# meilisearch/arroy

Measured on AMD Instinct MI355X. Metric: distances/sec, Q=1 batched 768-dim cosine scan (GB/s vs HBM roofline in `roofline`); tree-build seconds at 10M vectors in `build_10m`, higher is better.
Workload: dtype f32; 1 GPU; 1M x 768 cosine Q=1 scan (configs[1])

## Files before the change

### arroy_amd/csrc/dense_device.h

```cpp
#pragma once

namespace ah {

typedef _Float16 f16x8_t __attribute__((ext_vector_type(8)));
typedef float f32x16_t __attribute__((ext_vector_type(16)));
typedef float f32x4_t __attribute__((ext_vector_type(4)));

constexpr uint32_t kDM = 256;
template <int WN>
struct DenseShape {
    static constexpr uint32_t kBN = 64u * WN;
    static constexpr uint32_t kThreads = 128u * WN;
    static constexpr uint32_t kWaves = 2u * WN;
    static constexpr uint32_t kStage = (kDM + kBN) * 128u;
    static constexpr uint32_t kPiecesA = 32u / kWaves, kPiecesB = (kBN / 8u) / kWaves;
};
constexpr uint32_t kDenseHalf = 128;
constexpr uint32_t kDensePitch = kDM + 4;
constexpr uint32_t kDenseLds = kDenseHalf * kDensePitch * 4;
constexpr uint32_t kDenseGroup = 8;
static_assert(2 * DenseShape<4>::kStage <= kDenseLds && 2 * DenseShape<2>::kStage <= kDenseLds, "stage buffers fit");

constexpr uint32_t kSideUndecided = 2u;
constexpr uint32_t kSideVerify = 4u;

struct DenseArgs {
    const uint16_t *rows;
    const float4 *stats;
    const float *headers;
    uint64_t n;
    uint32_t hpitch;
    const uint8_t *shadow;
    uint64_t hstride;
    uint32_t n_cols;
    const FNode *nodes;
    const uint32_t *node_of;
    uint8_t *side_bytes;
    float gamma_s, gamma_r;
    uint32_t n_row_tiles, n_col_tiles, group, verify;
};

template <int WN>
__device__ __forceinline__ void dense_stage(const uint8_t *const (&a_src)[DenseShape<WN>::kPiecesA],
                                            const uint8_t *const (&b_src)[DenseShape<WN>::kPiecesB], uint32_t kb, uint8_t *stage,
                                            uint32_t wave) {
    typedef DenseShape<WN> SH;
    const uint64_t koff = (uint64_t)kb * 128u;
#pragma unroll
    for (uint32_t i = 0; i < SH::kPiecesA; i++)
        __builtin_amdgcn_global_load_lds((const __attribute__((address_space(1))) void *)(a_src[i] + koff),
                                         (__attribute__((address_space(3))) void *)(stage + (i * SH::kWaves + wave) * 1024u), 16, 0,
                                         0);
#pragma unroll
    for (uint32_t i = 0; i < SH::kPiecesB; i++)
        __builtin_amdgcn_global_load_lds(
            (const __attribute__((address_space(1))) void *)(b_src[i] + koff),
            (__attribute__((address_space(3))) void *)(stage + kDM * 128u + (i * SH::kWaves + wave) * 1024u), 16, 0, 0);
}

__device__ __forceinline__ bool dense_block_map(uint32_t b, uint32_t group, uint32_t n_col_tiles, uint32_t n_row_tiles,
                                                uint32_t &rt, uint32_t &ct) {
    const uint32_t xcd = b & 7u, slot = b >> 3;
    const uint32_t per_group = group * n_col_tiles;
    const uint32_t grp = slot / per_group, within = slot % per_group;
    ct = within / group;
    rt = (grp * group + within % group) * 8u + xcd;
    return rt < n_row_tiles;
}
__global__ void k_dense_coverage(uint32_t group, uint32_t n_col_tiles, uint32_t n_row_tiles, uint32_t *__restrict__ counts) {
    uint32_t rt, ct;
    if (!dense_block_map(blockIdx.x, group, n_col_tiles, n_row_tiles, rt, ct)) return;
    if (threadIdx.x == 0) atomicAdd(&counts[(uint64_t)rt * n_col_tiles + ct], 1u);
}

template <int METRIC, int WN>
__global__ __launch_bounds__(DenseShape<WN>::kThreads, 1) void k_forest_dense_screen(DenseArgs a, const AbortFlags abort_flag) {
    typedef DenseShape<WN> SH;
    extern __shared__ uint4 s_dense4[];
    uint8_t *smem = reinterpret_cast<uint8_t *>(s_dense4);
    if (abort_requested(abort_flag)) return;
    uint32_t rt, ct;
    if (!dense_block_map(blockIdx.x, a.group, a.n_col_tiles, a.n_row_tiles, rt, ct)) return;
    const uint64_t row0 = (uint64_t)rt * kDM;
    const uint32_t c0 = ct * SH::kBN;
    const uint32_t wave = threadIdx.x >> 6, lane = threadIdx.x & 63u;

    const uint8_t *a_src[SH::kPiecesA], *b_src[SH::kPiecesB];
    {
        const uint32_t sl = lane & 7u;
#pragma unroll
        for (uint32_t i = 0; i < SH::kPiecesA; i++) {
            const uint32_t R = (i * SH::kWaves + wave) * 8u + (lane >> 3);
            const uint64_t r = min(row0 + R, a.n - 1);
            a_src[i] = reinterpret_cast<const uint8_t *>(a.rows) + r * ((uint64_t)a.hpitch * 2u) + ((sl ^ ((R >> 1) & 7u)) << 4);
        }
#pragma unroll
        for (uint32_t i = 0; i < SH::kPiecesB; i++) {
            const uint32_t R = (i * SH::kWaves + wave) * 8u + (lane >> 3);
            const uint32_t c = min(c0 + R, a.n_cols - 1);
            b_src[i] = a.shadow + (uint64_t)c * a.hstride + ((sl ^ ((R >> 1) & 7u)) << 4);
        }
    }
    const uint32_t wm = wave / WN, wn = wave % WN;
    const uint32_t m = lane & 31u, g = lane >> 5, swz = (m >> 1) & 7u;
    f32x16_t acc[4][2];
#pragma unroll
    for (int im = 0; im < 4; im++)
#pragma unroll
        for (int jn = 0; jn < 2; jn++)
#pragma unroll
            for (int e = 0; e < 16; e++) acc[im][jn][e] = 0.0f;

    const uint32_t nk = a.hpitch >> 6;
    dense_stage<WN>(a_src, b_src, 0, smem, wave);
    for (uint32_t kb = 0; kb < nk; kb++) {
        asm volatile("s_waitcnt vmcnt(0)" ::: "memory");
        __syncthreads();
        if (kb + 1 < nk) dense_stage<WN>(a_src, b_src, kb + 1, smem + ((kb + 1) & 1u) * SH::kStage, wave);
        const uint8_t *st = smem + (kb & 1u) * SH::kStage;
        const uint8_t *sa = st + (wm * 128u + m) * 128u;
        const uint8_t *sb = st + (kDM + wn * 64u + m) * 128u;
#pragma unroll
        for (uint32_t q = 0; q < 4; q++) {
            const uint32_t off = ((2u * q + g) ^ swz) << 4;
            f16x8_t af[4], bf[2];
#pragma unroll
            for (int im = 0; im < 4; im++) af[im] = *reinterpret_cast<const f16x8_t *>(sa + im * 32 * 128 + off);
#pragma unroll
            for (int jn = 0; jn < 2; jn++) bf[jn] = *reinterpret_cast<const f16x8_t *>(sb + jn * 32 * 128 + off);
#pragma unroll
            for (int im = 0; im < 4; im++)
#pragma unroll
                for (int jn = 0; jn < 2; jn++)
                    acc[im][jn] = __builtin_amdgcn_mfma_f32_32x32x16_f16(af[im], bf[jn], acc[im][jn], 0, 0, 0);
        }
    }
    float *S = reinterpret_cast<float *>(smem);
    const uint32_t r_in = threadIdx.x & (kDM - 1u), part = threadIdx.x / kDM;
    constexpr uint32_t kParts = SH::kThreads / kDM;
    const uint64_t row = row0 + r_in;
    const bool live = row < a.n;
    float4 rs = make_float4(0.f, 0.f, 0.f, 0.f);
    float row_extra = 0.0f;
    if (live) {
        rs = a.stats[row];
        if (METRIC == AH_DOT_PRODUCT) row_extra = a.headers[2 * row];
    }
#pragma unroll 1
    for (uint32_t h = 0; h < SH::kBN / kDenseHalf; h++) {
        const uint32_t c_lo = c0 + h * kDenseHalf;
        if (c_lo >= a.n_cols) break;
        __syncthreads();
        if ((wn >> 1) == h) {
#pragma unroll
            for (int im = 0; im < 4; im++)
#pragma unroll
                for (int jn = 0; jn < 2; jn++) {
                    const uint32_t col = (wn & 1u) * 64u + (uint32_t)jn * 32u + m;
#pragma unroll
                    for (int qq = 0; qq < 4; qq++) {
                        const uint32_t rr = wm * 128u + (uint32_t)im * 32u + 8u * (uint32_t)qq + 4u * g;
                        *reinterpret_cast<float4 *>(S + col * kDensePitch + rr) = make_float4(
                            acc[im][jn][4 * qq], acc[im][jn][4 * qq + 1], acc[im][jn][4 * qq + 2], acc[im][jn][4 * qq + 3]);
                    }
                }
        }
        __syncthreads();
        const uint32_t c_hi = min(c_lo + kDenseHalf, a.n_cols) - 1u;
        const uint32_t t_lo = a.nodes[c_lo].tree, t_hi = a.nodes[c_hi].tree;
        for (uint32_t t = t_lo + 8u * part; t <= t_hi; t += 8u * kParts) {
            uint32_t nd[8];
#pragma unroll
            for (uint32_t u = 0; u < 8; u++)
                nd[u] = (live && t + u <= t_hi) ? a.node_of[(uint64_t)(t + u) * a.n + row] : 0xFFFFFFFFu;
#pragma unroll
            for (uint32_t u = 0; u < 8; u++) {
                const uint32_t c = nd[u] - c_lo;
                if (nd[u] != 0xFFFFFFFFu && c < kDenseHalf) {
                    const float s = S[c * kDensePitch + r_in];
                    const NormalStats ns =
                        *reinterpret_cast<const NormalStats *>(a.shadow + (uint64_t)nd[u] * a.hstride + (uint64_t)a.hpitch * 2u);
                    uint32_t side;
                    const bool decided = screen_decides<METRIC>(s, rs, ns, row_extra, a.gamma_s, a.gamma_r, side);
                    a.side_bytes[(uint64_t)(t + u) * a.n + row] =
                        (uint8_t)(decided ? (a.verify ? (kSideVerify | side) : side) : kSideUndecided);
                }
            }
        }
    }
}

#ifndef AH_NARROW_SETS
#define AH_NARROW_SETS 3u
#endif
#ifndef AH_NARROW_PRELOAD
#define AH_NARROW_PRELOAD 1
#endif
constexpr uint32_t kNarrowWaves = 5;
constexpr uint32_t kNarrowRows = 32u * kNarrowWaves;
constexpr uint32_t kNarrowThreads = 64u * (kNarrowWaves + 1u);
template <int NT>
struct NarrowShape {
    static constexpr uint32_t kCT = 32u * NT;
    static constexpr uint32_t kStage = kCT * 128u;
    static constexpr uint32_t kStages = 3;
    static constexpr uint32_t kPieces = kCT / 8u;
    static constexpr uint32_t kEpiWave = 32u * 36u * 4u;
    static constexpr uint32_t kRing = kStages * kStage > kNarrowWaves * kEpiWave ? kStages * kStage : kNarrowWaves * kEpiWave;
    static constexpr uint32_t kLds = kRing + kCT * 16u;
};

template <int METRIC, int NT, bool STREAM>
__global__ __launch_bounds__(kNarrowThreads, 2) void k_forest_dense_narrow(DenseArgs a, const AbortFlags abort_flag) {
    typedef NarrowShape<NT> SH;
    extern __shared__ uint4 s_dense4[];
    uint8_t *smem = reinterpret_cast<uint8_t *>(s_dense4);
    if (abort_requested(abort_flag)) return;
    uint32_t rt, ct;
    if (!dense_block_map(blockIdx.x, a.group, a.n_col_tiles, a.n_row_tiles, rt, ct)) return;
    const uint32_t wave = threadIdx.x >> 6, lane = threadIdx.x & 63u;
    const uint32_t c0 = ct * SH::kCT;
    const uint32_t nk = a.hpitch >> 6;
    if (wave == kNarrowWaves) {
        const uint8_t *b_src[SH::kPieces];
#pragma unroll
        for (uint32_t p = 0; p < SH::kPieces; p++) {
            const uint32_t R = p * 8u + (lane >> 3);
            const uint32_t c = min(c0 + R, a.n_cols - 1);
            b_src[p] = a.shadow + (uint64_t)c * a.hstride + (((lane & 7u) ^ ((R >> 1) & 7u)) << 4);
        }
        {
            NormalStats *nst_all = reinterpret_cast<NormalStats *>(smem + SH::kRing);
#pragma unroll
            for (uint32_t h = 0; h < SH::kCT / 64u; h++)
                nst_all[64u * h + lane] = *reinterpret_cast<const NormalStats *>(
                    a.shadow + (uint64_t)min(c0 + 64u * h + lane, a.n_cols - 1) * a.hstride + (uint64_t)a.hpitch * 2u);
        }
#define AH_NARROW_DMA(KB, SET)                                                                                            \
    _Pragma("unroll") for (uint32_t p_ = 0; p_ < SH::kPieces; p_++) __builtin_amdgcn_global_load_lds(                     \
        (const __attribute__((address_space(1))) void *)(b_src[p_] + (uint64_t)(KB) * 128u),                              \
        (__attribute__((address_space(3))) void *)(smem + (SET) * SH::kStage + p_ * 1024u), 16, 0, 0)
        AH_NARROW_DMA(0, 0);
        if (nk > 1) AH_NARROW_DMA(1, 1);
        for (uint32_t kb = 0; kb < nk; kb++) {
            if (kb + 1 < nk) asm volatile("s_waitcnt vmcnt(%0)" ::"n"(SH::kPieces) : "memory");
            else asm volatile("s_waitcnt vmcnt(0)" ::: "memory");
            __builtin_amdgcn_s_barrier();
            asm volatile("" ::: "memory");
            if (kb + 2 < nk) {
                const uint32_t set = (kb + 2) % 3u;
                AH_NARROW_DMA(kb + 2, set);
            }
        }
#undef AH_NARROW_DMA
        __builtin_amdgcn_s_barrier();
        return;
    }
    const uint32_t m = lane & 15u, kg = lane >> 4;
    const uint64_t row_base = (uint64_t)rt * kNarrowRows + wave * 32u;
    const uint4 *a_src[2];
#pragma unroll
    for (uint32_t i = 0; i < 2; i++)
        a_src[i] = reinterpret_cast<const uint4 *>(reinterpret_cast<const uint8_t *>(a.rows) +
                                                  min(row_base + 16u * i + m, a.n - 1) * ((uint64_t)a.hpitch * 2u) + 16u * kg);
    f32x4_t acc[2][2 * NT];
#pragma unroll
    for (int i = 0; i < 2; i++)
#pragma unroll
        for (int j = 0; j < 2 * NT; j++) acc[i][j] = f32x4_t{0.0f, 0.0f, 0.0f, 0.0f};
    const uint32_t er = lane & 31u, eh = lane >> 5;
    const uint64_t row = row_base + er;
    const bool live = row < a.n;
    float4 rs = make_float4(0.f, 0.f, 0.f, 0.f);
    float row_extra = 0.0f;
    const uint32_t T0 = a.nodes[c0].tree, T1 = a.nodes[min(c0 + SH::kCT, a.n_cols) - 1u].tree;
    uint32_t nd0[8];
#define AH_NARROW_LOAD_ND0()                                                                                              \
    _Pragma("unroll") for (uint32_t u = 0; u < 8; u++) {                                                                  \
        const uint32_t t = T0 + eh + 2u * u;                                                                              \
        const uint32_t v = a.node_of[(uint64_t)min(t, T1) * a.n + min(row, a.n - 1)];                                     \
        nd0[u] = (live && t <= T1) ? v : 0xFFFFFFFFu;        \
    }
    {
        const uint64_t r = min(row, a.n - 1);
        rs = a.stats[r];
        if (METRIC == AH_DOT_PRODUCT) row_extra = a.headers[2 * r];
    }
#if AH_NARROW_PRELOAD
    AH_NARROW_LOAD_ND0()
#endif
    constexpr uint32_t kSets = NT == 2 ? AH_NARROW_SETS : 3u, kAhead = kSets - 1u;
    uint4 ar[kSets][4];
#define AH_NARROW_ISSUE(KB, SET)                                                                                          \
    _Pragma("unroll") for (int i_ = 0; i_ < 4; i_++) ar[SET][i_] =                                                        \
        STREAM ? ld_stream_u4(a_src[i_ >> 1] + (uint64_t)(KB) * 8u + 4u * (i_ & 1))                                       \
               : a_src[i_ >> 1][(uint64_t)(KB) * 8u + 4u * (i_ & 1)]
#define AH_NARROW_STEP(SET, STEADY)                                                                                       \
    if (STEADY || kb + (SET) < nk) {                                                                                      \
        asm volatile("s_waitcnt lgkmcnt(0)" ::: "memory");              \
        __builtin_amdgcn_s_barrier();                                                                                     \
        asm volatile("" ::: "memory");                                                                                    \
        if (STEADY || kb + (SET) + kAhead < nk) AH_NARROW_ISSUE(kb + (SET) + kAhead, ((SET) + kAhead) % kSets);           \
        __builtin_amdgcn_sched_barrier(0);        \
        const uint8_t *sb_ = smem + ((kb + (SET)) % SH::kStages) * SH::kStage + m * 128u;                                 \
        _Pragma("unroll") for (uint32_t s_ = 0; s_ < 2; s_++) {                                                           \
            const f16x8_t a0_ = __builtin_bit_cast(f16x8_t, ar[SET][s_]);                                                 \
            const f16x8_t a1_ = __builtin_bit_cast(f16x8_t, ar[SET][2 + s_]);                                             \
            _Pragma("unroll") for (int j_ = 0; j_ < 2 * NT; j_++) {                                                       \
                                                  \
                const f16x8_t b_ = *reinterpret_cast<const f16x8_t *>(sb_ + j_ * 2048 + (((4u * s_ + kg) ^ ((m >> 1) & 7u)) << 4)); \
                acc[0][j_] = __builtin_amdgcn_mfma_f32_16x16x32_f16(a0_, b_, acc[0][j_], 0, 0, 0);                        \
                acc[1][j_] = __builtin_amdgcn_mfma_f32_16x16x32_f16(a1_, b_, acc[1][j_], 0, 0, 0);                        \
            }                                                                                                             \
        }                                                                                                                 \
    }
#pragma unroll
    for (uint32_t p = 0; p < kAhead; p++) AH_NARROW_ISSUE(min(p, nk - 1u), p);
    uint32_t kb = 0;
    for (; kb + 2u * kSets - 1u <= nk; kb += kSets) {
        AH_NARROW_STEP(0, true)
        AH_NARROW_STEP(1, true)
        AH_NARROW_STEP(2, true)
        if (kSets == 4) AH_NARROW_STEP(kSets - 1, true)
    }
    for (; kb < nk; kb += kSets) {
        AH_NARROW_STEP(0, false)
        AH_NARROW_STEP(1, false)
        AH_NARROW_STEP(2, false)
        if (kSets == 4) AH_NARROW_STEP(kSets - 1, false)
    }
#undef AH_NARROW_STEP
#undef AH_NARROW_ISSUE
    asm volatile("s_waitcnt lgkmcnt(0)" ::: "memory");
    __builtin_amdgcn_s_barrier();
    asm volatile("" ::: "memory");
#if !AH_NARROW_PRELOAD
    AH_NARROW_LOAD_ND0()
#endif
#undef AH_NARROW_LOAD_ND0
    float *S = reinterpret_cast<float *>(smem + wave * SH::kEpiWave);
    const NormalStats *nst_all = reinterpret_cast<const NormalStats *>(smem + SH::kRing);
// ... 156 lines not shown
```

### arroy_amd/csrc/forest.hip

```cpp
#include <algorithm>
#include <atomic>
#include <chrono>
#include <condition_variable>
#include <deque>
#include <array>
#include <thread>
#include <type_traits>
#include <unordered_map>
#include <cstdlib>
#include <immintrin.h>
#include <sys/mman.h>
#include <sys/syscall.h>
#include <unistd.h>
#include <new>

#include "common.h"
#include "split_device.h"
#include "screen_device.h"
#include "level_plan.h"
#include "encode.h"
#include "node_codec.h"

namespace ah {

// ... 2187 lines not shown
            }
            cv.notify_all();
        }
        if (ev[0]) (void)hipEventDestroy(ev[0]);
        if (ev[1]) (void)hipEventDestroy(ev[1]);
        if (cs) (void)hipStreamDestroy(cs);
    }
    void push(void *dst, const void *src, size_t bytes) {
        if (!bytes) return;
        if (inline_mode) {
            const hipError_t e = hipMemcpy(dst, src, bytes, hipMemcpyDeviceToHost);
            if (e != hipSuccess && err == hipSuccess) err = e;
            return;
        }
        {
            std::lock_guard<std::mutex> lk(mu);
            q.push_back(Job{dst, src, bytes, nullptr});
            pending++;
        }
        cv.notify_all();
    }
    void push_stream(StreamJob *job, const void *src) {
        if (job->nodes.empty()) {
            delete job;
            return;
        }
        if (inline_mode) {
            hipStream_t cs = nullptr;
            hipEvent_t ev[2] = {nullptr, nullptr};
            hipError_t e = create_copy_stream(&cs);
            if (e == hipSuccess) e = hipEventCreateWithFlags(&ev[0], hipEventDisableTiming);
            if (e == hipSuccess) e = hipEventCreateWithFlags(&ev[1], hipEventDisableTiming);
            if (e == hipSuccess) e = deliver(*job, reinterpret_cast<const uint8_t *>(src), cs, ev);
            if (e != hipSuccess && err == hipSuccess) err = e;
            if (ev[0]) (void)hipEventDestroy(ev[0]);
            if (ev[1]) (void)hipEventDestroy(ev[1]);
            if (cs) (void)hipStreamDestroy(cs);
            delete job;
            return;
        }
        {
            std::lock_guard<std::mutex> lk(mu);
            q.push_back(Job{nullptr, src, 1, job});
            pending++;
        }
        cv.notify_all();
    }
    hipError_t drain() {
        std::unique_lock<std::mutex> lk(mu);
        cv.wait(lk, [this] { return pending == 0; });
        return err;
    }
    ~Readback() {
        if (!started) return;
        {
            std::lock_guard<std::mutex> lk(mu);
            stop = true;
        }
        cv.notify_all();
        th.join();
    }
};

namespace {
struct LevelBufs {
    DataView dv;
    ScreenView sv;
    int metric, device;
    hipStream_t s;
    uint64_t N;
    uint32_t n_trees, n_nodes, n_tiles;
    FNode *nodes;
    FTile *tiles;
    uint32_t *perm;
    uint8_t *normals;
    uint64_t nstride, hdr_off;
    uint8_t *shadow;
    uint64_t hstride;
    uint8_t *shadow8;
    uint64_t stride8;
    uint64_t *masks;
    uint32_t *tile_left, *node_of;
    uint8_t *side_bytes;
    uint32_t *side_bits;
    ScreenCounters *counters;
    AbortFlags abort_all, abort_gated;
    uint32_t verify;
};

template <class F>
int with_metric(int metric, F &&f) {
    return with_metric_of<AH_EUCLIDEAN, AH_MANHATTAN, AH_COSINE, AH_DOT_PRODUCT>(metric, f);
}

int launch_create_split(const LevelBufs &b, int metric, unsigned grid, size_t cs_shared) {
    return with_metric(metric, [&](auto m) -> int {
        constexpr int M = decltype(m)::value;
        AH_TRY(lds_opt_in(reinterpret_cast<const void *>(k_forest_create_split<M>), b.device, cs_shared));
        hipLaunchKernelGGL(k_forest_create_split<M>, dim3(grid), dim3(64), cs_shared, b.s, b.dv, b.nodes, b.n_nodes, b.perm, b.N,
                           b.normals, b.nstride, b.hdr_off, b.abort_gated.gate);
        return AH_OK;
    });
}

template <int M, int TC, bool LDS>
int launch_screen_rows_inst(const LevelBufs &b, const RowsLaunch &l, const RowsSchedule &sch, unsigned grid, size_t sh, size_t lds_grant) {
    const unsigned threads = LDS ? (TC >= 16 ? 512u : 1024u) : (unsigned)kBlock;
    if (LDS) AH_TRY(lds_opt_in(reinterpret_cast<const void *>(k_forest_screen_rows<M, TC, LDS>), b.device, lds_grant));
    hipLaunchKernelGGL((k_forest_screen_rows<M, TC, LDS>), dim3(grid), dim3(threads), LDS ? sh : 0, b.s, b.dv, b.sv, b.node_of,
                       l.t0, l.np, b.normals, b.nstride, b.hdr_off, b.shadow, b.hstride, b.side_bytes, sch, b.abort_all,
                       b.counters, b.verify);
    return AH_OK;
}
int launch_screen_rows(const LevelBufs &b, const RowsLaunch &l, bool lds, const RowsSchedule &sch, unsigned grid, size_t sh,
                       size_t lds_grant) {
    return with_metric(b.metric, [&](auto m) -> int {
        constexpr int M = decltype(m)::value;
        if (lds) return l.tcv >= 16 ? launch_screen_rows_inst<M, 16, true>(b, l, sch, grid, sh, lds_grant)
                                    : launch_screen_rows_inst<M, 8, true>(b, l, sch, grid, sh, lds_grant);
        switch (l.tcv) {
        case 16: return launch_screen_rows_inst<M, 16, false>(b, l, sch, grid, sh, lds_grant);
        case 8: return launch_screen_rows_inst<M, 8, false>(b, l, sch, grid, sh, lds_grant);
        case 4: return launch_screen_rows_inst<M, 4, false>(b, l, sch, grid, sh, lds_grant);
        default: return launch_screen_rows_inst<M, 2, false>(b, l, sch, grid, sh, lds_grant);
        }
    });
}
}

namespace {
struct DensePlan {
    uint32_t n_row_tiles, n_col_tiles, group;
    bool wide;
    int narrow;
    bool stream;
    uint32_t tile_rows, tile_cols, threads, lds;
    uint64_t grid;
};
DensePlan dense_plan(uint64_t N, uint32_t n_cols) {
    DensePlan p{};
    const long long narrow_max = tun(TUN_DENSE_NARROW_MAX_COLS), narrow_force = tun(TUN_DENSE_NARROW);
    p.narrow = narrow_force == 0 || (long long)n_cols > narrow_max ? 0 : (n_cols <= 64 ? 2 : 4);
    if (p.narrow) {
        p.tile_rows = kNarrowRows;
        p.tile_cols = 32u * (uint32_t)p.narrow;
        p.threads = kNarrowThreads;
        p.lds = p.narrow == 2 ? NarrowShape<2>::kLds : NarrowShape<4>::kLds;
        p.wide = false;
    } else {
        p.wide = n_cols > 128;
        p.tile_rows = kDM;
        p.tile_cols = p.wide ? 256u : 128u;
        p.threads = p.wide ? DenseShape<4>::kThreads : DenseShape<2>::kThreads;
        p.lds = kDenseLds;
    }
    p.n_row_tiles = (uint32_t)((N + p.tile_rows - 1) / p.tile_rows);
    p.n_col_tiles = (n_cols + p.tile_cols - 1) / p.tile_cols;
    p.group = p.n_col_tiles > 1 ? (p.narrow ? 12u : kDenseGroup) : 1u;
    const long long st = tun(TUN_DENSE_NARROW_STREAM);
    p.stream = p.narrow && (st < 0 ? p.n_col_tiles == 1 : st != 0);
    const uint64_t r8 = (p.n_row_tiles + 7) / 8;
    p.grid = 8 * ((r8 + p.group - 1) / p.group) * p.group * p.n_col_tiles;
    return p;
}
unsigned exact_pairs_grid(uint64_t N, uint32_t n_trees) {
    return (unsigned)std::min<uint64_t>((((N + 1023) / 1024 + 7) / 8) * 8 * ((n_trees + 3) / 4), 1u << 16);
}
}

namespace {
struct RowsPlan {
    RowsSchedule sch{};
    unsigned threads = kBlock;
    bool xcd = false, nt = false;
    std::vector<std::pair<uint32_t, unsigned>> launches;
};
int plan_rows_launches(uint64_t N, uint32_t hpitch, uint32_t tcv, uint32_t groups, bool lds, uint64_t group_normal_bytes,
                       RowsPlan *plan) {
    const uint32_t env_rpb = (uint32_t)std::max<long long>(0, tun(TUN_ROWS_PER_BLOCK)) / 32u * 32u;
    const uint32_t rpb = lds ? 1024u : env_rpb ? env_rpb : 32u;
    const uint64_t hrow = (uint64_t)hpitch * 2;
    const uint64_t want_rows = tun(TUN_ROWS_CHUNK_ROWS) > 0 ? (uint64_t)tun(TUN_ROWS_CHUNK_ROWS)
                                                             : ((uint64_t)std::max<long long>(1, tun(TUN_ROWS_CHUNK_MB)) << 20) / hrow;
    uint32_t chunk_rows = (uint32_t)std::max<uint64_t>(rpb, want_rows / rpb * rpb);
    if (chunk_rows > N) chunk_rows = (uint32_t)((N + rpb - 1) / rpb * rpb);
    const uint32_t n_chunks = (uint32_t)((N + chunk_rows - 1) / chunk_rows);
    RowsSchedule &sch = plan->sch;
    sch.n_groups = groups;
    sch.tiles = chunk_rows / rpb;
    sch.chunk_rows = chunk_rows;
    sch.rows_per_block = rpb;
    plan->xcd = !lds && tun(TUN_ROWS_XCD) != 0 && tcv <= 4 && groups >= (uint32_t)std::max<long long>(1, tun(TUN_ROWS_XCD_MIN_GROUPS));
    sch.xcd_slots = plan->xcd ? (groups + 7) / 8 : 0u;
    const uint64_t per_chunk = plan->xcd ? 8ull * sch.xcd_slots * sch.tiles : (uint64_t)groups * sch.tiles;
    const long long nt_force = tun(TUN_ROWS_NT);
    plan->nt = plan->xcd && (nt_force >= 0 ? nt_force != 0 : group_normal_bytes > (uint64_t)std::max<long long>(0, tun(TUN_ROWS_NT_BYTES)));
    if (plan->nt) sch.xcd_slots |= 0x80000000u;
    plan->threads = lds ? (tcv >= 16 ? 512u : 1024u) : (unsigned)kBlock;
    const uint64_t max_items = (uint64_t)std::min<long long>(0xFFFFFFFFll, std::max<long long>(1, tun(TUN_LAUNCH_MAX_ITEMS)));
    AH_REQUIRE(per_chunk * plan->threads <= max_items, AH_ERR_INVALID_ARGUMENT, "forest build: too many trees for one row-major launch");
    const uint32_t chunks_per_launch = (uint32_t)std::min<uint64_t>(n_chunks, (max_items / plan->threads) / per_chunk);
    plan->launches.clear();
    for (uint32_t c0 = 0; c0 < n_chunks; c0 += chunks_per_launch)
        plan->launches.emplace_back(c0, (unsigned)((uint64_t)std::min<uint32_t>(chunks_per_launch, n_chunks - c0) * per_chunk));
    return AH_OK;
}
}

namespace {
template <int M, int WN>
int launch_dense_wide(const LevelBufs &b, const DensePlan &dp, const DenseArgs &da) {
    AH_TRY(lds_opt_in(reinterpret_cast<const void *>(k_forest_dense_screen<M, WN>), b.device, kDenseLds));
    hipLaunchKernelGGL((k_forest_dense_screen<M, WN>), dim3((unsigned)dp.grid), dim3(DenseShape<WN>::kThreads), kDenseLds, b.s, da,
                       b.abort_all);
    return AH_OK;
}
template <int M, int NT>
int launch_dense_narrow(const LevelBufs &b, const DensePlan &dp, const DenseArgs &da) {
    if (dp.stream)
        hipLaunchKernelGGL((k_forest_dense_narrow<M, NT, true>), dim3((unsigned)dp.grid), dim3(kNarrowThreads), NarrowShape<NT>::kLds,
                           b.s, da, b.abort_all);
    else
        hipLaunchKernelGGL((k_forest_dense_narrow<M, NT, false>), dim3((unsigned)dp.grid), dim3(kNarrowThreads), NarrowShape<NT>::kLds,
                           b.s, da, b.abort_all);
    return AH_OK;
}
int launch_dense(const LevelBufs &b, const DensePlan &dp, bool exact_wide, ah_build_stats &st) {
    DenseArgs da{};
    da.rows = b.sv.rows;
    da.stats = b.sv.stats;
    da.headers = b.dv.headers;
    da.n = b.N;
    da.hpitch = b.sv.hpitch;
    da.shadow = b.shadow;
    da.hstride = b.hstride;
    da.n_cols = b.n_nodes;
    da.nodes = b.nodes;
    da.node_of = b.node_of;
    da.side_bytes = b.side_bytes;
    da.gamma_s = (float)(2.0 * ((double)b.sv.hpitch + (double)b.sv.hpitch / 16 + 16.0) * 1.1920929e-7);
    da.gamma_r = b.sv.gamma_r;
    da.n_row_tiles = dp.n_row_tiles;
    da.n_col_tiles = dp.n_col_tiles;
    da.group = dp.group;
    da.verify = b.verify;
    AH_REQUIRE(dp.grid < 0x7FFFFFFFull, AH_ERR_INVALID_ARGUMENT, "forest build: too many tiles for one launch");
    const unsigned egrid = exact_pairs_grid(b.N, b.n_trees);
    AH_TRY(with_metric(b.metric, [&](auto m) -> int {
        constexpr int M = decltype(m)::value;
        if (dp.narrow == 2) AH_TRY((launch_dense_narrow<M, 2>(b, dp, da)));
        else if (dp.narrow == 4) AH_TRY((launch_dense_narrow<M, 4>(b, dp, da)));
        else if (dp.wide) AH_TRY((launch_dense_wide<M, 4>(b, dp, da)));
        else AH_TRY((launch_dense_wide<M, 2>(b, dp, da)));
        if (exact_wide)
            hipLaunchKernelGGL((k_forest_exact_pairs<M, true>), dim3(egrid), dim3(256), 0, b.s, b.dv, b.node_of, b.side_bytes,
                               b.n_trees, b.normals, b.nstride, b.hdr_off, b.counters, b.abort_all);
        else
            hipLaunchKernelGGL((k_forest_exact_pairs<M>), dim3(egrid), dim3(256), 0, b.s, b.dv, b.node_of, b.side_bytes, b.n_trees,
                               b.normals, b.nstride, b.hdr_off, b.counters, b.abort_all);
        return AH_OK;
    }));
    st.dense_launches++;
    st.dense_columns += b.n_nodes;
    return AH_OK;
}

int launch_rows_screened(const LevelBufs &b, const LevelPlan &plan, uint64_t nodes_per_tree, uint64_t rec_bytes,
                         const uint32_t *d_tree_first, size_t lds_grant, ah_build_stats &st) {
    const bool lds = plan.lds_tc != 0;
    const size_t lds_sh = (size_t)plan.lds_worst * rec_bytes;
    for (const RowsLaunch &l : plan.launches) {
        RowsPlan rp;
        AH_TRY(plan_rows_launches(b.N, b.sv.hpitch, l.tcv, l.groups, lds, (uint64_t)l.tcv * nodes_per_tree * rec_bytes, &rp));
        rp.sch.tree_first = d_tree_first;
        for (const auto &c : rp.launches) {
            rp.sch.chunk0 = c.first;
            AH_TRY(launch_screen_rows(b, l, lds, rp.sch, c.second, lds_sh, lds_grant));
        }
        st.margin_mode_launches[lds ? (l.tcv >= 16 ? MM_LDS16 : MM_LDS8) : mm_rows(l.tcv)]++;
        st.rows_xcd_launches += rp.xcd ? rp.launches.size() : 0;
        st.rows_nt_launches += rp.nt ? rp.launches.size() : 0;
        st.rows_split_launches += rp.launches.size() - 1;
    }
    return AH_OK;
}

template <int M, int TC>
int launch_rows_lds_inst(const LevelBufs &b, uint32_t t0, uint32_t np, uint32_t first, uint32_t cnt, size_t sh, size_t lds_grant) {
    const unsigned per_cu = (unsigned)std::max<size_t>(1, std::min<size_t>(2, (150u << 10) / std::max<size_t>(sh, 1)));
    const unsigned threads = TC >= 16 ? 512u : 1024u;
    const unsigned grid = (unsigned)std::min<uint64_t>((b.N * 8 + threads - 1) / threads, 256u * per_cu);
    AH_TRY(lds_opt_in(reinterpret_cast<const void *>(k_forest_margin_rows_lds<M, TC>), b.device, lds_grant));
    hipLaunchKernelGGL((k_forest_margin_rows_lds<M, TC>), dim3(grid), dim3(threads), sh, b.s, b.dv, b.node_of, t0, np, b.normals,
                       b.nstride, b.hdr_off, b.side_bytes, first, cnt, b.abort_all);
    return AH_OK;
}
template <int M, int TC>
int launch_rows_inst(const LevelBufs &b, uint32_t t0, uint32_t np, unsigned row_grid) {
    hipLaunchKernelGGL((k_forest_margin_rows<M, TC>), dim3(row_grid), dim3(kBlock), 0, b.s, b.dv, b.node_of, t0, np, b.normals,
                       b.nstride, b.hdr_off, b.side_bytes, b.abort_all);
    return AH_OK;
}
int launch_rows_f32(const LevelBufs &b, const LevelPlan &plan, uint64_t rec_bytes, unsigned row_grid, size_t lds_grant,
                    ah_build_stats &st) {
    for (const RowsLaunch &l : plan.launches)
        for (uint32_t g = 0; g < l.groups; g++) {
            const uint32_t t0 = l.t0 + g * l.tcv;
            if (plan.lds_tc) {
                const uint32_t first = plan.tree_first[t0], cnt = plan.tree_first[t0 + l.np] - first;
                if (cnt == 0) continue;
                const size_t sh = (size_t)cnt * rec_bytes;
                AH_TRY(with_metric(b.metric, [&](auto m) -> int {
                    constexpr int M = decltype(m)::value;
                    return l.tcv >= 16 ? launch_rows_lds_inst<M, 16>(b, t0, l.np, first, cnt, sh, lds_grant)
                                       : launch_rows_lds_inst<M, 8>(b, t0, l.np, first, cnt, sh, lds_grant);
                }));
                st.margin_mode_launches[l.tcv >= 16 ? MM_LDS16 : MM_LDS8]++;
            } else {
                AH_TRY(with_metric(b.metric, [&](auto m) -> int {
                    constexpr int M = decltype(m)::value;
                    switch (l.tcv) {
                    case 16: return launch_rows_inst<M, 16>(b, t0, l.np, row_grid);
                    case 8: return launch_rows_inst<M, 8>(b, t0, l.np, row_grid);
                    case 4: return launch_rows_inst<M, 4>(b, t0, l.np, row_grid);
                    default: return launch_rows_inst<M, 2>(b, t0, l.np, row_grid);
                    }
                }));
                st.margin_mode_launches[mm_rows(l.tcv)]++;
            }
        }
    return AH_OK;
}

int launch_node_major(const LevelBufs &b, bool bq, bool screen, bool screen8, bool node_pre, unsigned node_grid, ah_build_stats &st) {
    if (bq) {
        hipLaunchKernelGGL(k_forest_margin_bq, dim3(node_grid), dim3(kBlock), b.dv.pitch * 8, b.s, b.dv, b.nodes, b.tiles, b.n_tiles,
                           b.perm, b.N, b.normals, b.nstride, b.hdr_off, b.masks, b.tile_left, b.abort_gated);
        st.margin_mode_launches[MM_BQ]++;
        return AH_OK;
    }
    if (screen) {
        const size_t sh = (size_t)b.dv.pitch * 4 + (size_t)b.sv.hpitch * 2 + (screen8 ? 2 * (size_t)b.sv.pitch8 : 0);
        auto launch = [&](auto m, auto pre) -> int {
            constexpr int M = decltype(m)::value, PRE = decltype(pre)::value;
            AH_TRY(lds_opt_in(reinterpret_cast<const void *>(k_forest_screen_node<M, PRE>), b.device, sh));
            hipLaunchKernelGGL((k_forest_screen_node<M, PRE>), dim3(node_grid), dim3(kBlock), sh, b.s, b.dv, b.sv, b.nodes, b.tiles,
                               b.n_tiles, b.perm, b.normals, b.nstride, b.hdr_off, b.shadow, b.hstride, b.shadow8, b.stride8, b.masks,
                               b.tile_left, b.abort_gated, b.counters, b.verify);
            return AH_OK;
        };
        AH_TRY(with_metric(b.metric, [&](auto m) -> int {
            return node_pre ? launch(m, std::integral_constant<int, 6>{}) : launch(m, std::integral_constant<int, 0>{});
        }));
        st.margin_mode_launches[MM_NODE]++;
        st.screened_launches++;
        return AH_OK;
    }
    const size_t sh = (size_t)b.dv.pitch * 4;
    AH_TRY(with_metric(b.metric, [&](auto m) -> int {
        constexpr int M = decltype(m)::value;
        AH_TRY(lds_opt_in(reinterpret_cast<const void *>(k_forest_margin_f32<M>), b.device, sh));
        hipLaunchKernelGGL((k_forest_margin_f32<M>), dim3(node_grid), dim3(kBlock), sh, b.s, b.dv, b.nodes, b.tiles, b.n_tiles, b.perm,
                           b.N, b.normals, b.nstride, b.hdr_off, b.masks, b.tile_left, b.abort_gated);
        return AH_OK;
    }));
    st.margin_mode_launches[MM_NODE]++;
// ... 1585 lines not shown
```

Baseline: 3.066 billion distances/s.

## Pipeline dense screen k-loop in half-tile phases with staggered waves and LDS-staged stats

```diff
diff --git a/arroy_amd/csrc/dense_device.h b/arroy_amd/csrc/dense_device.h
--- a/arroy_amd/csrc/dense_device.h
+++ b/arroy_amd/csrc/dense_device.h
@@ -1,12 +1,20 @@
 #pragma once
+#include "dense_schedule.h"
 
 namespace ah {
+
+#ifndef AH_DENSE_STAGGER
+#define AH_DENSE_STAGGER 1
+#endif
 
 typedef _Float16 f16x8_t __attribute__((ext_vector_type(8)));
 typedef float f32x16_t __attribute__((ext_vector_type(16)));
 typedef float f32x4_t __attribute__((ext_vector_type(4)));
 
 constexpr uint32_t kDM = 256;
+constexpr uint32_t kDenseHalf = 128;
+constexpr uint32_t kDensePitch = kDM + 4;
+constexpr uint32_t kDenseLds = kDenseHalf * kDensePitch * 4;
 template <int WN>
 struct DenseShape {
     static constexpr uint32_t kBN = 64u * WN;
@@ -14,10 +22,15 @@
     static constexpr uint32_t kWaves = 2u * WN;
     static constexpr uint32_t kStage = (kDM + kBN) * 128u;
     static constexpr uint32_t kPiecesA = 32u / kWaves, kPiecesB = (kBN / 8u) / kWaves;
+    static constexpr uint32_t kHalfA = kPiecesA / 2u, kHalfB = kPiecesB / 2u;
+    static constexpr uint32_t kWaitSteady = dense_wait_steady(kHalfA, kHalfB);
+    static_assert(kWaitSteady == kHalfA + 2u * kHalfB && dense_schedule_ok_to(13, kHalfA, kHalfB), "dense_schedule.h");
+    static constexpr uint32_t kLdsNormalStats = kDenseLds;
+    static constexpr uint32_t kLdsRowStats = kLdsNormalStats + kBN * 16u;
+    static constexpr uint32_t kLdsRowExtra = kLdsRowStats + kDM * 16u;
+    static constexpr uint32_t kLds = kLdsRowExtra + kDM * 4u;
+    static_assert(kLds <= 160u * 1024u && kWaves * 64u >= kDM && kBN <= kDM, "LDS of one block; a lane per row in dense_stage_aux");
 };
-constexpr uint32_t kDenseHalf = 128;
-constexpr uint32_t kDensePitch = kDM + 4;
-constexpr uint32_t kDenseLds = kDenseHalf * kDensePitch * 4;
 constexpr uint32_t kDenseGroup = 8;
 static_assert(2 * DenseShape<4>::kStage <= kDenseLds && 2 * DenseShape<2>::kStage <= kDenseLds, "stage buffers fit");
 
@@ -41,21 +54,70 @@
 };
 
 template <int WN>
-__device__ __forceinline__ void dense_stage(const uint8_t *const (&a_src)[DenseShape<WN>::kPiecesA],
-                                            const uint8_t *const (&b_src)[DenseShape<WN>::kPiecesB], uint32_t kb, uint8_t *stage,
-                                            uint32_t wave) {
+__device__ __forceinline__ constexpr uint32_t dense_piece_a(uint32_t h, uint32_t i, uint32_t wave) {
+    const uint32_t q = i * DenseShape<WN>::kWaves + wave;
+    return (q >> 3) * 16u + h * 8u + (q & 7u);
+}
+template <int WN>
+__device__ __forceinline__ constexpr uint32_t dense_piece_b(uint32_t h, uint32_t i, uint32_t wave) {
+    const uint32_t q = i * DenseShape<WN>::kWaves + wave;
+    return (q >> 2) * 8u + h * 4u + (q & 3u);
+}
+template <int WN, uint32_t J>
+__device__ __forceinline__ void dense_stage_half(const uint8_t *const (&a_src)[2][DenseShape<WN>::kHalfA],
+                                                 const uint8_t *const (&b_src)[2][DenseShape<WN>::kHalfB], uint32_t kb,
+                                                 uint8_t *stage, uint32_t wave) {
     typedef DenseShape<WN> SH;
     const uint64_t koff = (uint64_t)kb * 128u;
-#pragma unroll
-    for (uint32_t i = 0; i < SH::kPiecesA; i++)
-        __builtin_amdgcn_global_load_lds((const __attribute__((address_space(1))) void *)(a_src[i] + koff),
-                                         (__attribute__((address_space(3))) void *)(stage + (i * SH::kWaves + wave) * 1024u), 16, 0,
-                                         0);
-#pragma unroll
-    for (uint32_t i = 0; i < SH::kPiecesB; i++)
+    if (J == kHalfA0 || J == kHalfA1) {
+        constexpr uint32_t h = J == kHalfA1;
+#pragma unroll
+        for (uint32_t i = 0; i < SH::kHalfA; i++)
+            __builtin_amdgcn_global_load_lds((const __attribute__((address_space(1))) void *)(a_src[h][i] + koff),
+                                             (__attribute__((address_space(3))) void *)(stage + dense_piece_a<WN>(h, i, wave) * 1024u),
+                                             16, 0, 0);
+    } else {
+        constexpr uint32_t h = J == kHalfB1;
+#pragma unroll
+        for (uint32_t i = 0; i < SH::kHalfB; i++)
+            __builtin_amdgcn_global_load_lds(
+                (const __attribute__((address_space(1))) void *)(b_src[h][i] + koff),
+                (__attribute__((address_space(3))) void *)(stage + kDM * 128u + dense_piece_b<WN>(h, i, wave) * 1024u), 16, 0, 0);
+    }
+}
+template <int METRIC, int WN>
+__device__ __forceinline__ void dense_stage_aux(const DenseArgs &a, uint64_t row0, uint32_t c0, uint8_t *smem, uint32_t wave,
+                                                uint32_t lane) {
+    typedef DenseShape<WN> SH;
+    if (wave < SH::kBN / 64u) {
+        const uint32_t c = min(c0 + 64u * wave + lane, a.n_cols - 1u);
         __builtin_amdgcn_global_load_lds(
-            (const __attribute__((address_space(1))) void *)(b_src[i] + koff),
-            (__attribute__((address_space(3))) void *)(stage + kDM * 128u + (i * SH::kWaves + wave) * 1024u), 16, 0, 0);
+            (const __attribute__((address_space(1))) void *)(a.shadow + (uint64_t)c * a.hstride + (uint64_t)a.hpitch * 2u),
+            (__attribute__((address_space(3))) void *)(smem + SH::kLdsNormalStats + wave * 1024u), 16, 0, 0);
+    }
+    if (wave >= SH::kWaves - kDM / 64u) {
+        const uint32_t w = wave - (SH::kWaves - kDM / 64u);
+        const uint64_t r = min(row0 + 64u * w + lane, a.n - 1);
+        __builtin_amdgcn_global_load_lds((const __attribute__((address_space(1))) void *)(a.stats + r),
+                                         (__attribute__((address_space(3))) void *)(smem + SH::kLdsRowStats + w * 1024u), 16, 0, 0);
+        if (METRIC == AH_DOT_PRODUCT)
+            __builtin_amdgcn_global_load_lds((const __attribute__((address_space(1))) void *)(a.headers + 2u * r),
+                                             (__attribute__((address_space(3))) void *)(smem + SH::kLdsRowExtra + w * 256u), 4, 0, 0);
+    }
+}
+template <uint32_t N>
+__device__ __forceinline__ void dense_wait_dma() {
+    asm volatile("s_waitcnt vmcnt(%0)" ::"n"(N) : "memory");
+}
+__device__ __forceinline__ void dense_reads_done_barrier() {
+    asm volatile("s_waitcnt lgkmcnt(0)" ::: "memory");
+    __builtin_amdgcn_s_barrier();
+    asm volatile("" ::: "memory");
+}
+__device__ __forceinline__ void dense_raw_barrier() {
+    asm volatile("" ::: "memory");
+    __builtin_amdgcn_s_barrier();
+    asm volatile("" ::: "memory");
 }
 
 __device__ __forceinline__ bool dense_block_map(uint32_t b, uint32_t group, uint32_t n_col_tiles, uint32_t n_row_tiles,
@@ -85,20 +147,23 @@
     const uint32_t c0 = ct * SH::kBN;
     const uint32_t wave = threadIdx.x >> 6, lane = threadIdx.x & 63u;
 
-    const uint8_t *a_src[SH::kPiecesA], *b_src[SH::kPiecesB];
+    const uint8_t *a_src[2][SH::kHalfA], *b_src[2][SH::kHalfB];
     {
         const uint32_t sl = lane & 7u;
 #pragma unroll
-        for (uint32_t i = 0; i < SH::kPiecesA; i++) {
-            const uint32_t R = (i * SH::kWaves + wave) * 8u + (lane >> 3);
-            const uint64_t r = min(row0 + R, a.n - 1);
-            a_src[i] = reinterpret_cast<const uint8_t *>(a.rows) + r * ((uint64_t)a.hpitch * 2u) + ((sl ^ ((R >> 1) & 7u)) << 4);
-        }
-#pragma unroll
-        for (uint32_t i = 0; i < SH::kPiecesB; i++) {
-            const uint32_t R = (i * SH::kWaves + wave) * 8u + (lane >> 3);
-            const uint32_t c = min(c0 + R, a.n_cols - 1);
-            b_src[i] = a.shadow + (uint64_t)c * a.hstride + ((sl ^ ((R >> 1) & 7u)) << 4);
+        for (uint32_t h = 0; h < 2; h++) {
+#pragma unroll
+            for (uint32_t i = 0; i < SH::kHalfA; i++) {
+                const uint32_t R = dense_piece_a<WN>(h, i, wave) * 8u + (lane >> 3);
+                const uint64_t r = min(row0 + R, a.n - 1);
+                a_src[h][i] = reinterpret_cast<const uint8_t *>(a.rows) + r * ((uint64_t)a.hpitch * 2u) + ((sl ^ ((R >> 1) & 7u)) << 4);
+            }
+#pragma unroll
+            for (uint32_t i = 0; i < SH::kHalfB; i++) {
+                const uint32_t R = dense_piece_b<WN>(h, i, wave) * 8u + (lane >> 3);
+                const uint32_t c = min(c0 + R, a.n_cols - 1);
+                b_src[h][i] = a.shadow + (uint64_t)c * a.hstride + ((sl ^ ((R >> 1) & 7u)) << 4);
+            }
         }
     }
     const uint32_t wm = wave / WN, wn = wave % WN;
@@ -111,43 +176,101 @@
 #pragma unroll
             for (int e = 0; e < 16; e++) acc[im][jn][e] = 0.0f;
 
+    constexpr uint32_t kRounds = SH::kBN / kDenseHalf;
+    uint32_t t_lo[kRounds], t_hi[kRounds];
+#pragma unroll
+    for (uint32_t h = 0; h < kRounds; h++) {
+        const uint32_t c_lo = min(c0 + h * kDenseHalf, a.n_cols - 1u), c_hi = min(c0 + (h + 1u) * kDenseHalf, a.n_cols) - 1u;
+        t_lo[h] = a.nodes[c_lo].tree;
+        t_hi[h] = a.nodes[max(c_lo, c_hi)].tree;
+    }
+
     const uint32_t nk = a.hpitch >> 6;
-    dense_stage<WN>(a_src, b_src, 0, smem, wave);
-    for (uint32_t kb = 0; kb < nk; kb++) {
-        asm volatile("s_waitcnt vmcnt(0)" ::: "memory");
-        __syncthreads();
-        if (kb + 1 < nk) dense_stage<WN>(a_src, b_src, kb + 1, smem + ((kb + 1) & 1u) * SH::kStage, wave);
-        const uint8_t *st = smem + (kb & 1u) * SH::kStage;
-        const uint8_t *sa = st + (wm * 128u + m) * 128u;
-        const uint8_t *sb = st + (kDM + wn * 64u + m) * 128u;
-#pragma unroll
-        for (uint32_t q = 0; q < 4; q++) {
-            const uint32_t off = ((2u * q + g) ^ swz) << 4;
-            f16x8_t af[4], bf[2];
-#pragma unroll
-            for (int im = 0; im < 4; im++) af[im] = *reinterpret_cast<const f16x8_t *>(sa + im * 32 * 128 + off);
-#pragma unroll
-            for (int jn = 0; jn < 2; jn++) bf[jn] = *reinterpret_cast<const f16x8_t *>(sb + jn * 32 * 128 + off);
-#pragma unroll
-            for (int im = 0; im < 4; im++)
-#pragma unroll
-                for (int jn = 0; jn < 2; jn++)
-                    acc[im][jn] = __builtin_amdgcn_mfma_f32_32x32x16_f16(af[im], bf[jn], acc[im][jn], 0, 0, 0);
-        }
-    }
+    dense_stage_aux<METRIC, WN>(a, row0, c0, smem, wave, lane);
+    dense_stage_half<WN, kHalfA0>(a_src, b_src, 0, smem, wave);
+    dense_stage_half<WN, kHalfB0>(a_src, b_src, 0, smem, wave);
+    dense_stage_half<WN, kHalfB1>(a_src, b_src, 0, smem, wave);
+    dense_stage_half<WN, kHalfA1>(a_src, b_src, 0, smem, wave);
+    if (nk > 1) {
+        dense_stage_half<WN, kHalfA0>(a_src, b_src, 1, smem + SH::kStage, wave);
+        dense_stage_half<WN, kHalfB0>(a_src, b_src, 1, smem + SH::kStage, wave);
+        dense_stage_half<WN, kHalfB1>(a_src, b_src, 1, smem + SH::kStage, wave);
+        dense_wait_dma<SH::kWaitSteady>();
+    } else {
+        dense_wait_dma<0>();
+    }
+    dense_raw_barrier();
+    if (AH_DENSE_STAGGER && wm == 1) dense_raw_barrier();
+    const uint32_t a_off = (wm * 128u + m) * 128u, b_off = (kDM + wn * 64u + m) * 128u;
+    for (uint32_t t = 0; t < nk; t++) {
+        uint8_t *st = smem + (t & 1u) * SH::kStage, *st_next = smem + ((t + 1u) & 1u) * SH::kStage;
+        const uint8_t *sa = st + a_off, *sb = st + b_off;
+        const bool more1 = t + 1u < nk, more2 = t + 2u < nk;
+        f16x8_t af[2][4], bf[2][4];
+#define AH_DENSE_READ_A(H)                                                                                                \
+    _Pragma("unroll") for (uint32_t q = 0; q < 4; q++) _Pragma("unroll") for (uint32_t i = 0; i < 2; i++) af[i][q] =       \
+        *reinterpret_cast<const f16x8_t *>(sa + (2u * (H) + i) * 32u * 128u + (((2u * q + g) ^ swz) << 4))
+#define AH_DENSE_READ_B(H)                                                                                                \
+    _Pragma("unroll") for (uint32_t q = 0; q < 4; q++) bf[H][q] =                                                          \
+        *reinterpret_cast<const f16x8_t *>(sb + (H) * 32u * 128u + (((2u * q + g) ^ swz) << 4))
+#define AH_DENSE_MFMA(HA, HB)                                                                                             \
+    __builtin_amdgcn_s_setprio(1);                                                                                        \
+    _Pragma("unroll") for (uint32_t q = 0; q < 4; q++) _Pragma("unroll") for (uint32_t i = 0; i < 2; i++)                  \
+        acc[2 * (HA) + i][HB] = __builtin_amdgcn_mfma_f32_32x32x16_f16(af[i][q], bf[HB][q], acc[2 * (HA) + i][HB], 0, 0, 0); \
+    __builtin_amdgcn_s_setprio(0)
+        AH_DENSE_READ_B(0);
+        AH_DENSE_READ_A(0);
+        if (more1) dense_stage_half<WN, kHalfA1>(a_src, b_src, t + 1u, st_next, wave);
+        dense_reads_done_barrier();
+        AH_DENSE_MFMA(0, 0);
+        dense_raw_barrier();
+        AH_DENSE_READ_B(1);
+        if (more2) dense_stage_half<WN, kHalfA0>(a_src, b_src, t + 2u, st, wave);
+        dense_reads_done_barrier();
+        AH_DENSE_MFMA(0, 1);
+        dense_raw_barrier();
+        AH_DENSE_READ_A(1);
+        if (more2) dense_stage_half<WN, kHalfB0>(a_src, b_src, t + 2u, st, wave);
+        dense_reads_done_barrier();
+        AH_DENSE_MFMA(1, 1);
+        dense_raw_barrier();
+        if (more2) {
+            dense_stage_half<WN, kHalfB1>(a_src, b_src, t + 2u, st, wave);
+            dense_wait_dma<SH::kWaitSteady>();
+        } else if (more1) {
+            dense_wait_dma<0>();
+        }
+        dense_reads_done_barrier();
+        AH_DENSE_MFMA(1, 0);
+        dense_raw_barrier();
+#undef AH_DENSE_READ_A
+#undef AH_DENSE_READ_B
+#undef AH_DENSE_MFMA
+    }
+    if (AH_DENSE_STAGGER && wm == 0) dense_raw_barrier();
     float *S = reinterpret_cast<float *>(smem);
     const uint32_t r_in = threadIdx.x & (kDM - 1u), part = threadIdx.x / kDM;
     constexpr uint32_t kParts = SH::kThreads / kDM;
-    const uint64_t row = row0 + r_in;
+    const uint64_t row = row0 + r_in, row_c = min(row, a.n - 1);
     const bool live = row < a.n;
-    float4 rs = make_float4(0.f, 0.f, 0.f, 0.f);
-    float row_extra = 0.0f;
-    if (live) {
-        rs = a.stats[row];
-        if (METRIC == AH_DOT_PRODUCT) row_extra = a.headers[2 * row];
-    }
-#pragma unroll 1
-    for (uint32_t h = 0; h < SH::kBN / kDenseHalf; h++) {
+    uint32_t nd0[kRounds][8];
+#pragma unroll
+    for (uint32_t h = 0; h < kRounds; h++) {
+#pragma unroll
+        for (uint32_t u = 0; u < 8; u++)
+            nd0[h][u] = a.node_of[(uint64_t)min(t_lo[h] + 8u * part + u, t_hi[h]) * a.n + row_c];
+    }
+    __builtin_amdgcn_sched_barrier(0);
+#pragma unroll
+    for (uint32_t h = 0; h < kRounds; h++)
+#pragma unroll
+        for (uint32_t u = 0; u < 8; u++)
+            if (!(live && t_lo[h] + 8u * part + u <= t_hi[h])) nd0[h][u] = 0xFFFFFFFFu;
+    const float4 rs = reinterpret_cast<const float4 *>(smem + SH::kLdsRowStats)[r_in];
+    const float row_extra = METRIC == AH_DOT_PRODUCT ? reinterpret_cast<const float *>(smem + SH::kLdsRowExtra)[r_in] : 0.0f;
+    const NormalStats *nst = reinterpret_cast<const NormalStats *>(smem + SH::kLdsNormalStats);
+#pragma unroll
+    for (uint32_t h = 0; h < kRounds; h++) {
         const uint32_t c_lo = c0 + h * kDenseHalf;
         if (c_lo >= a.n_cols) break;
         __syncthreads();
@@ -166,27 +289,31 @@
                 }
         }
         __syncthreads();
-        const uint32_t c_hi = min(c_lo + kDenseHalf, a.n_cols) - 1u;
-        const uint32_t t_lo = a.nodes[c_lo].tree, t_hi = a.nodes[c_hi].tree;
-        for (uint32_t t = t_lo + 8u * part; t <= t_hi; t += 8u * kParts) {
+#define AH_DENSE_DECIDE(T, NODE)                                                                                          \
+    do {                                                                                                                  \
+        const uint32_t node_ = (NODE), c_ = node_ - c_lo;                                                                 \
+        if (node_ != 0xFFFFFFFFu && c_ < kDenseHalf) {                                                                    \
+            uint32_t side_;                                                                                               \
+            const bool decided_ = screen_decides<METRIC>(S[c_ * kDensePitch + r_in], rs, nst[node_ - c0], row_extra,      \
+                                                         a.gamma_s, a.gamma_r, side_);                                    \
+            a.side_bytes[(uint64_t)(T) * a.n + row] =                                                                     \
+                (uint8_t)(decided_ ? (a.verify ? (kSideVerify | side_) : side_) : kSideUndecided);                        \
+        }                                                                                                                 \
+    } while (0)
+#pragma unroll
+        for (uint32_t u = 0; u < 8; u++) AH_DENSE_DECIDE(t_lo[h] + 8u * part + u, nd0[h][u]);
+        for (uint32_t t = t_lo[h] + 8u * (part + kParts); t <= t_hi[h]; t += 8u * kParts) {
             uint32_t nd[8];
 #pragma unroll
+            for (uint32_t u = 0; u < 8; u++) nd[u] = a.node_of[(uint64_t)min(t + u, t_hi[h]) * a.n + row_c];
+            __builtin_amdgcn_sched_barrier(0);
+#pragma unroll
             for (uint32_t u = 0; u < 8; u++)
-                nd[u] = (live && t + u <= t_hi) ? a.node_of[(uint64_t)(t + u) * a.n + row] : 0xFFFFFFFFu;
-#pragma unroll
-            for (uint32_t u = 0; u < 8; u++) {
-                const uint32_t c = nd[u] - c_lo;
-                if (nd[u] != 0xFFFFFFFFu && c < kDenseHalf) {
-                    const float s = S[c * kDensePitch + r_in];
-                    const NormalStats ns =
-                        *reinterpret_cast<const NormalStats *>(a.shadow + (uint64_t)nd[u] * a.hstride + (uint64_t)a.hpitch * 2u);
-                    uint32_t side;
-                    const bool decided = screen_decides<METRIC>(s, rs, ns, row_extra, a.gamma_s, a.gamma_r, side);
-                    a.side_bytes[(uint64_t)(t + u) * a.n + row] =
-                        (uint8_t)(decided ? (a.verify ? (kSideVerify | side) : side) : kSideUndecided);
-                }
-            }
-        }
+                if (!(live && t + u <= t_hi[h])) nd[u] = 0xFFFFFFFFu;
+#pragma unroll
+            for (uint32_t u = 0; u < 8; u++) AH_DENSE_DECIDE(t + u, nd[u]);
+        }
+#undef AH_DENSE_DECIDE
     }
 }
 
diff --git a/arroy_amd/csrc/dense_schedule.h b/arroy_amd/csrc/dense_schedule.h
--- /dev/null
+++ b/arroy_amd/csrc/dense_schedule.h
@@ -0,0 +1,95 @@
+#pragma once
+#include <cstdint>
+
+namespace ah {
+
+constexpr uint32_t kDensePhases = 4;
+constexpr uint32_t kDenseAhead = 7;
+constexpr uint32_t kDenseInFlight = 3;
+
+enum DenseHalf : uint32_t { kHalfA0 = 0, kHalfB0 = 1, kHalfB1 = 2, kHalfA1 = 3 };
+
+constexpr uint32_t dense_half_pieces(uint32_t j, uint32_t pa, uint32_t pb) { return (j == kHalfA0 || j == kHalfA1) ? pa : pb; }
+constexpr uint32_t dense_half_read_phase(uint32_t j) { return j == kHalfA0 || j == kHalfB0 ? 0u : j == kHalfB1 ? 1u : 2u; }
+
+constexpr uint32_t dense_wait_count(uint32_t n_kblocks, int32_t t, uint32_t pa, uint32_t pb) {
+    const uint32_t n_half = kDensePhases * n_kblocks, first = kDensePhases * (uint32_t)(t + 2);
+    uint32_t n = 0;
+    for (uint32_t s = first; s < first + kDenseInFlight && s < n_half; s++) n += dense_half_pieces(s % kDensePhases, pa, pb);
+    return n;
+}
+constexpr uint32_t dense_wait_steady(uint32_t pa, uint32_t pb) { return dense_wait_count(64, 0, pa, pb); }
+
+constexpr int dense_schedule_check(uint32_t n_kblocks, uint32_t pa, uint32_t pb, bool stagger) {
+    constexpr uint32_t kMax = 32 * kDensePhases;
+    if (n_kblocks == 0 || n_kblocks * kDensePhases > kMax) return 5;
+    const uint32_t n_half = kDensePhases * n_kblocks;
+    const int64_t kNever = -1000000;
+    int64_t landed_at[kMax] = {};
+    int64_t last_read_at[2][4] = {};
+    bool region_full[2][4] = {};
+    uint32_t queue[kMax] = {}, q_head = 0, q_tail = 0, in_flight = 0, issued = 0;
+    for (uint32_t s = 0; s < kMax; s++) landed_at[s] = -kNever;
+    for (uint32_t b = 0; b < 2; b++)
+        for (uint32_t j = 0; j < 4; j++) last_read_at[b][j] = kNever;
+    const int64_t late = stagger ? 1 : 0;
+    auto issue = [&](uint32_t s, int64_t passed_first) -> int {
+        if (s != issued) return 5;
+        const uint32_t b = (s / kDensePhases) & 1u, j = s % kDensePhases;
+        if (region_full[b][j]) return 2;
+        if (!(last_read_at[b][j] < passed_first)) return 2;
+        region_full[b][j] = true;
+        queue[q_tail++] = s;
+        in_flight += dense_half_pieces(j, pa, pb);
+        issued++;
+        return 0;
+    };
+    auto wait = [&](uint32_t n, int64_t passed_last) -> int {
+        if (n > 63) return 6;
+        while (in_flight > n) {
+            const uint32_t s = queue[q_head++];
+            in_flight -= dense_half_pieces(s % kDensePhases, pa, pb);
+            landed_at[s] = passed_last;
+        }
+        return 0;
+    };
+    for (uint32_t s = 0; s < kDenseAhead && s < n_half; s++)
+        if (int e = issue(s, -1)) return e;
+    if (int e = wait(dense_wait_count(n_kblocks, -1, pa, pb), -1)) return e;
+    for (uint32_t ph = 0; ph < n_half; ph++) {
+        const uint32_t t = ph / kDensePhases, p = ph % kDensePhases;
+        const int64_t first = 2 * (int64_t)ph, last = first + late;
+        for (uint32_t j = 0; j < 4; j++) {
+            if (dense_half_read_phase(j) != p) continue;
+            const uint32_t s = kDensePhases * t + j;
+            if (!region_full[t & 1u][j] || !(landed_at[s] < first)) return 1;
+            region_full[t & 1u][j] = false;
+            last_read_at[t & 1u][j] = last;
+        }
+        if (ph + kDenseAhead < n_half)
+            if (int e = issue(ph + kDenseAhead, first)) return e;
+        if (p == kDensePhases - 1 && t + 1 < n_kblocks) {
+            const uint32_t n = dense_wait_count(n_kblocks, (int32_t)t, pa, pb);
+            if (n == 0 && t + 2 < n_kblocks) return 4;
+            if (int e = wait(n, last)) return e;
+        }
+    }
+    if (in_flight != 0 || issued != n_half) return 3;
+    for (uint32_t b = 0; b < 2; b++)
+        for (uint32_t j = 0; j < 4; j++)
+            if (region_full[b][j]) return 5;
+    return 0;
+}
+
+constexpr bool dense_schedule_ok_to(uint32_t n_max, uint32_t pa, uint32_t pb) {
+    for (uint32_t nk = 1; nk <= n_max; nk++)
+        if (dense_schedule_check(nk, pa, pb, false) != 0 || dense_schedule_check(nk, pa, pb, true) != 0) return false;
+    return true;
+}
+static_assert(dense_schedule_ok_to(13, 2, 2) && dense_schedule_ok_to(13, 4, 2), "k-loop schedule of k_forest_dense_screen");
+static_assert(dense_wait_steady(2, 2) == 6 && dense_wait_steady(4, 2) == 8, "loads per half-tile x half-tiles in flight");
+static_assert(dense_wait_count(1, -1, 2, 2) == 0 && dense_wait_count(2, -1, 2, 2) == 6 && dense_wait_count(2, 0, 2, 2) == 0 &&
+                  dense_wait_count(3, 0, 2, 2) == 6 && dense_wait_count(3, 1, 2, 2) == 0,
+              "prologue and drain");
+
+}
diff --git a/arroy_amd/csrc/forest.hip b/arroy_amd/csrc/forest.hip
--- a/arroy_amd/csrc/forest.hip
+++ b/arroy_amd/csrc/forest.hip
@@ -2363,7 +2363,7 @@
         p.tile_rows = kDM;
         p.tile_cols = p.wide ? 256u : 128u;
         p.threads = p.wide ? DenseShape<4>::kThreads : DenseShape<2>::kThreads;
-        p.lds = kDenseLds;
+        p.lds = p.wide ? DenseShape<4>::kLds : DenseShape<2>::kLds;
     }
     p.n_row_tiles = (uint32_t)((N + p.tile_rows - 1) / p.tile_rows);
     p.n_col_tiles = (n_cols + p.tile_cols - 1) / p.tile_cols;
@@ -2421,8 +2421,8 @@
 namespace {
 template <int M, int WN>
 int launch_dense_wide(const LevelBufs &b, const DensePlan &dp, const DenseArgs &da) {
-    AH_TRY(lds_opt_in(reinterpret_cast<const void *>(k_forest_dense_screen<M, WN>), b.device, kDenseLds));
-    hipLaunchKernelGGL((k_forest_dense_screen<M, WN>), dim3((unsigned)dp.grid), dim3(DenseShape<WN>::kThreads), kDenseLds, b.s, da,
+    AH_TRY(lds_opt_in(reinterpret_cast<const void *>(k_forest_dense_screen<M, WN>), b.device, DenseShape<WN>::kLds));
+    hipLaunchKernelGGL((k_forest_dense_screen<M, WN>), dim3((unsigned)dp.grid), dim3(DenseShape<WN>::kThreads), DenseShape<WN>::kLds, b.s, da,
                        b.abort_all);
     return AH_OK;
 }
```

After: 2.979 billion distances/s. 0.971x the previous value.
